# elizabethfong/SparkSmithWaterman

Hardware: NVIDIA B200
Metric: GCUPS incl. traceback (150 bp reads x 10k RefSeq-shaped refs per B200) (higher is better)
Workload: dtype s16x2

## Files before the change

sparksmithwaterman_b200/csrc/swb_trace_tile.cu:

```cuda
#include "swb_internal.h"
#include "swb_device.cuh"

#include <algorithm>
#include <cstdlib>

namespace swb {

namespace {

constexpr int NT = 128;
constexpr int TRACE_ROLL_K = 25;

template <int K> struct TileGeo {
    static constexpr int ROWW = Geo<K>::KW / 4;
    static constexpr int COLS = CB + 1;
    static constexpr int TILE_WORDS = ROWW * COLS;
    static constexpr int PROF_WORDS = 5 * GL * Geo<K>::KS;
};

template <int K>
__device__ __forceinline__ int tile_byte(const uint8_t *tile8, int rr, int cc)
{
    return tile8[(size_t)((cc * TileGeo<K>::ROWW + (rr >> 2)) * NT) * 4 + (rr & 3)];
}

template <int K>
__device__ __forceinline__ void store_col8(uint32_t *col, int top, const int (&H)[K], uint32_t k64k)
{
    constexpr int ROWW = TileGeo<K>::ROWW;
#pragma unroll
    for (int w = 0; w < ROWW; ++w) {
        const uint32_t v0 = (w == 0) ? (uint32_t)top : (uint32_t)H[4 * w - 1 < K ? 4 * w - 1 : 0];
        const uint32_t v1 = (4 * w + 0 < K) ? (uint32_t)H[4 * w + 0 < K ? 4 * w + 0 : 0] : 0u;
        const uint32_t v2 = (4 * w + 1 < K) ? (uint32_t)H[4 * w + 1 < K ? 4 * w + 1 : 0] : 0u;
        const uint32_t v3 = (4 * w + 2 < K) ? (uint32_t)H[4 * w + 2 < K ? 4 * w + 2 : 0] : 0u;
        const uint32_t p01 = v1 * k64k + ((w == 0 || 4 * w - 1 < K) ? v0 : 0u);
        const uint32_t p23 = v3 * k64k + v2;
        col[w * NT] = __byte_perm(p01, p23, 0x6420);
    }
}

__device__ __forceinline__ uint32_t prmt(uint32_t a, uint32_t b, uint32_t sel)
{
    uint32_t r;
    asm("prmt.b32 %0, %1, %2, %3;" : "=r"(r) : "r"(a), "r"(b), "r"(sel));
    return r;
}

template <int K, bool TIE_GT>
__global__ void __launch_bounds__(NT) tile_trace_kernel(const BatchParams P, const uint64_t *keys, uint32_t n_cells,
                                                        int chunk, int32_t *beginnings, int32_t *op_lens, uint32_t *ops,
                                                        int ops_stride, uint32_t k64k)
{
    using G = Geo<K>;
    using TG = TileGeo<K>;
    constexpr int KS = G::KS, ROWW = TG::ROWW;
    constexpr unsigned FULL = 0xffffffffu;
    extern __shared__ __align__(16) uint32_t smem[];
    __shared__ uint32_t seg_next;
    int *prof = reinterpret_cast<int *>(smem);
    uint32_t *tile = smem + TG::PROF_WORDS + threadIdx.x;
    const uint8_t *tile8 = reinterpret_cast<const uint8_t *>(tile);
    uint8_t *rcodes_s = reinterpret_cast<uint8_t *>(smem + TG::PROF_WORDS + (size_t)TG::TILE_WORDS * NT);
    const int gap = P.gap, match = P.match, mismatch = P.mismatch, sbias = P.seam_bias;
    const int ag = -gap;
    const uint32_t kone = k64k >> 16;

    const uint32_t c_lo = blockIdx.x * (uint32_t)chunk;
    const uint32_t c_hi = min(n_cells, c_lo + (uint32_t)chunk);
    uint32_t seg_lo = c_lo;
    while (seg_lo < c_hi) {
        const uint32_t slot = (uint32_t)(key_pair(keys[seg_lo]) / (uint64_t)P.n_refs);
        uint32_t seg_hi;
        {
            const uint64_t target = make_key((uint64_t)(slot + 1) * (uint64_t)P.n_refs, 0, 0);
            uint32_t lo = seg_lo, hi = c_hi;
            while (lo < hi) { const uint32_t mid = lo + ((hi - lo) >> 1); if (keys[mid] < target) lo = mid + 1; else hi = mid; }
            seg_hi = lo;
        }
        const int read_idx = P.rp_reads[slot];
        const int rh = (int)(slot & 1u);
        const int64_t roff = P.read_off[read_idx];
        const int m = (int)(P.read_off[read_idx + 1] - roff);
        __syncthreads();
        for (int idx = threadIdx.x; idx < 5 * GL * K; idx += NT) {
            const int cc = idx / (GL * K), rem = idx - cc * GL * K;
            const int tt = rem / K, r = rem - tt * K;
            const int row = tt * K + r;
            int s = S_PAD;
            if (row < m && cc < 4) s = ((int)P.read_codes[roff + row] == cc) ? match : mismatch;
            prof[(cc < 4 ? tt * 4 + cc : 4 * GL + tt) * KS + r] = s + ag;
        }
        for (int idx = threadIdx.x; idx < GL * K; idx += NT)
            rcodes_s[idx] = idx < m ? P.read_codes[roff + idx] : (uint8_t)0xFE;
        if (threadIdx.x == 0) seg_next = seg_lo;
        __syncthreads();

        bool busy = false;
        int ci = 0, cj = 0, n = 0;
        const uint32_t *rw = P.ref_words;
        int64_t bk = 0;
        uint32_t w_cell = 0, w_opword = 0;
        int w_h = 0, w_beg = 0, w_len = 0;

        for (;;) {
            if (!busy) {
                const uint32_t e = atomicAdd(&seg_next, 1u);
                if (e < seg_hi) {
                    const uint64_t key = keys[e];
                    const int ro = (int)(key_pair(key) - (uint64_t)slot * (uint64_t)P.n_refs);
                    const int ref = P.ref_sorted_of[ro];
                    ci = (int)key_i(key); cj = (int)key_j(key);
                    n = P.ref_len[ref];
                    rw = P.ref_words + P.ref_word_off[ref];
                    bk = (int64_t)(slot >> 1) * P.blocks_per_rp + P.ref_blk_off[ref];
                    w_cell = e; w_opword = 0; w_beg = 0; w_len = 0;
                    w_h = P.scores[(int64_t)ro * P.n_reads + read_idx];
                    busy = w_h > 0;
                    if (!busy) { beginnings[e] = 0; op_lens[e] = 0; }
                }
            }
            if (!__any_sync(FULL, busy)) break;

            const int t = busy ? (ci - 1) / K : 0;
            const int step = cj - 1 + t;
            const int b = busy ? step / CB : 0;
            int H[K], diag = 0;
            {
                load_checkpoint<K>(rec_lane<K>(P.rec, bk + b, t), busy && b > 0, [&](int w, uint32_t v) {
                    if (w < K) H[w < K ? w : 0] = half_of(v, rh); else diag = half_of(v, rh);
                });
            }
            int top[CB];
            {
                const uint32_t *sq = rec_lane<K>(P.rec, bk + b, t) + G::CKP * REC_P;
                const bool ld = busy && t > 0;
                const int bias0 = sbias * (9 - t);
#pragma unroll
                for (int p = 0; p < CB / 8; ++p) {
                    uint32_t v[8] = {0, 0, 0, 0, 0, 0, 0, 0};
                    if (ld) ldg256(sq + p * REC_P, v);
#pragma unroll
                    for (int e = 0; e < 8; ++e)
                        top[8 * p + e] = ld ? half_of(v[e], rh) - (bias0 + sbias * (8 * p + e)) : 0;
                }
            }
            uint32_t win; int ulo, uhi;
            {
                const int j0 = b * CB - t;
                const int wi = j0 >> 4;
                const uint32_t a0 = (busy && wi >= 0 && wi * 16 < n) ? __ldg(rw + wi) : 0u;
                const uint32_t a1 = (busy && wi + 1 >= 0 && (wi + 1) * 16 < n) ? __ldg(rw + wi + 1) : 0u;
                win = __funnelshift_r(a0, a1, 2 * (j0 & 15));
                ulo = -j0; uhi = busy ? n - j0 - 1 : -1;
            }
            store_col8<K>(tile, diag, H, k64k);

            const int *pbase = prof + t * 4 * KS, *ppad = prof + (4 * GL + t) * KS;
            auto column = [&](int u, int tv, uint32_t code) {
                const bool real = (u >= ulo) && (u <= uhi);
                const int *pv = real ? pbase + code * KS : ppad;
                int sv[G::KP];
                {
                    const int4 *p4 = reinterpret_cast<const int4 *>(pv);
#pragma unroll
                    for (int q = 0; q < G::KP / 4; ++q) {
                        const int4 v = p4[q];
                        sv[4 * q] = v.x; sv[4 * q + 1] = v.y; sv[4 * q + 2] = v.z; sv[4 * q + 3] = v.w;
                    }
                }
                const int floorc = ag * (u + 1);
                const int topb = tv + floorc;
                int nw = diag, nn = topb;
#pragma unroll
                for (int r = 0; r < K; ++r) {
                    const int tt = nw * (int)kone + sv[r];
                    const int pre = __vimax3_s32(tt, H[r], floorc);
                    nw = H[r];
                    H[r] = __viaddmax_s32(nn, gap, pre);
                    nn = H[r];
                }
                diag = topb;
                store_col8<K>(tile + (u + 1) * ROWW * NT, topb, H, k64k);
            };
            if constexpr (K < TRACE_ROLL_K) {
#pragma unroll
                for (int u = 0; u < CB; ++u) column(u, top[u], (win >> (2 * u)) & 3u);
            } else {
#pragma unroll 1
                for (int q = 0; q < CB / 4; ++q) {
                    int tv[4];
#pragma unroll
                    for (int e = 0; e < 4; ++e) {
                        int x = top[e];
#pragma unroll
                        for (int qq = 1; qq < CB / 4; ++qq) x = (q == qq) ? top[4 * qq + e] : x;
                        tv[e] = x;
                    }
                    const uint32_t wq = win >> (8 * q);
#pragma unroll
                    for (int e = 0; e < 4; ++e) column(4 * q + e, tv[e], (wq >> (2 * e)) & 3u);
                }
            }

            if (busy) {
                constexpr int UPB = NT * 4, COLB = ROWW * NT * 4;
                int r = ci - t * K;
                int c = step - b * CB + 1;
                const int cbase = cj - c;
                const uint8_t *pw = tile8 + (size_t)((c * ROWW + (r >> 2)) * NT) * 4;
                uint32_t sel3 = (uint32_t)(r & 3) + 3u;
                uint32_t wsh = __brev(win);
                wsh = ((wsh & 0x55555555u) << 1) | ((wsh >> 1) & 0x55555555u);
                wsh >>= 2 * (CB - c);
                const uint8_t *qp = rcodes_s + (ci - 1);
                uint32_t *op_ptr = ops + (size_t)w_cell * ops_stride + (w_len >> 4);
                uint32_t sh = 2u * ((uint32_t)w_len & 15u);
                int lastc = c;
                for (;;) {
                    const uint32_t w_c = *reinterpret_cast<const uint32_t *>(pw), u_c = *reinterpret_cast<const uint32_t *>(pw - UPB);
                    const uint32_t w_l = *reinterpret_cast<const uint32_t *>(pw - COLB), u_l = *reinterpret_cast<const uint32_t *>(pw - COLB - UPB);
                    const int hn = (int)prmt(u_c, w_c, sel3), hw = (int)prmt(u_l, w_l, sel3 + 1u), hnw = (int)prmt(u_l, w_l, sel3);
                    const int sc = ((uint32_t)*qp == (wsh & 3u)) ? match : mismatch;
                    const int whb = w_h + ag * c;
                    const bool eq_a = ((hnw + sc + ag - whb) & 0xff) == 0, eq_i = ((hn + gap - whb) & 0xff) == 0,
                               eq_d = ((hw - whb) & 0xff) == 0;
                    const uint32_t op = TIE_GT ? (eq_d ? 3u : (eq_i ? 2u : 1u)) : (eq_a ? 1u : (eq_i ? 2u : 3u));
                    lastc = c;
                    w_opword |= op << sh;
                    sh = (sh + 2u) & 31u;
                    if (sh == 0u) { *op_ptr = w_opword; w_opword = 0; }
                    op_ptr += (sh == 0u);
                    ++w_len;
                    w_h -= (op == 1u) ? sc : gap;
                    const int up = op != 3u, left = op != 2u;
                    r -= up; qp -= up; sel3 -= up;
                    if (sel3 < 3u) { sel3 = 6u; pw -= UPB; }
                    c -= left; pw -= left ? COLB : 0; wsh >>= 2 * left;
                    if (w_h <= 0 || r == 0 || c == 0) break;
                }
                ci = t * K + r; cj = cbase + c;
                w_beg = cbase + lastc;
                if (w_h <= 0) {
                    if (sh) *op_ptr = w_opword;
                    beginnings[w_cell] = w_beg;
                    op_lens[w_cell] = w_len;
                    busy = false;
                }
            }
        }
        seg_lo = seg_hi;
    }
}

template <int K> struct RowMask { using type = uint32_t; };
template <> struct RowMask<40> { using type = uint64_t; };
template <> struct RowMask<48> { using type = uint64_t; };
template <> struct RowMask<56> { using type = uint64_t; };
template <> struct RowMask<64> { using type = uint64_t; };
__device__ __forceinline__ int mask_ffs(uint32_t m) { return __ffs((int)m); }
__device__ __forceinline__ int mask_ffs(uint64_t m) { return __ffsll((long long)m); }

template <int K>
struct TileSweep {
    using mask_t = typename RowMask<K>::type;
    static_assert(K <= 8 * (int)sizeof(mask_t), "row mask too narrow for K");
    int rc[K], H[K];
    int diag, S, t, b;
    uint32_t win;
    mask_t rowok;
    int ulo, uhi;
    const uint32_t *sq;
    bool has_top;
    uint64_t pkey;
    int64_t pair;

    __device__ __forceinline__ void setup(const BatchParams &P, const TileTask &T, bool live)
    {
        using G = Geo<K>;
        const int rp = (int)(T.rp_half >> 1), rh = (int)(T.rp_half & 1u), ref = (int)T.ref_sorted;
        t = (int)T.lane; b = (int)T.block;
        S = 0x7fffffff; pkey = 0; pair = 0; diag = 0; win = 0; rowok = 0; ulo = 0; uhi = -1;
        sq = P.rec; has_top = false;
#pragma unroll
        for (int r = 0; r < K; ++r) { rc[r] = 0xFE; H[r] = 0; }
        if (!live) return;
        const int read_idx = P.rp_reads[2 * rp + rh];
        const int64_t off = P.read_off[read_idx];
        const int m = (int)(P.read_off[read_idx + 1] - off);
        const int n = P.ref_len[ref];
        const int64_t ro = P.ref_orig[ref];
        pair = ro * P.n_reads + read_idx;
        S = P.scores[pair];
        pkey = (uint64_t)T.rp_half * (uint64_t)P.n_refs + (uint64_t)ro;
#pragma unroll
        for (int r = 0; r < K; ++r) {
            const int row = t * K + r;
            rc[r] = (row < m) ? (int)P.read_codes[off + row] : 0xFE;
            if (row < m) rowok |= (mask_t)1 << r;
        }
        const int64_t blk = (int64_t)rp * P.blocks_per_rp + P.ref_blk_off[ref] + b;
        if (b > 0) {
            load_checkpoint<K>(rec_lane<K>(P.rec, blk, t), true, [&](int w, uint32_t v) {
                if (w < K) H[w < K ? w : 0] = half_of(v, rh); else diag = half_of(v, rh);
            });
        }
        sq = rec_lane<K>(P.rec, blk, t) + G::CKP * REC_P;
        has_top = t > 0;
        const uint32_t *rw = P.ref_words + P.ref_word_off[ref];
        const int j0 = b * CB - t;
        const int wi = j0 >> 4;
        const uint32_t a0 = (wi >= 0 && wi * 16 < n) ? __ldg(rw + wi) : 0u;
        const uint32_t a1 = (wi + 1 >= 0 && (wi + 1) * 16 < n) ? __ldg(rw + wi + 1) : 0u;
        win = __funnelshift_r(a0, a1, 2 * (j0 & 15));
        ulo = -j0; uhi = n - j0 - 1;
        (void)rh;
    }

    template <class Fn>
    __device__ __forceinline__ void run(const BatchParams &P, int rh, Fn &&fn)
    {
        const int gap = P.gap, match = P.match, mismatch = P.mismatch;
        const int bias0 = P.seam_bias * (9 - t);
        uint32_t sv[CB];
#pragma unroll
        for (int p = 0; p < CB / 8; ++p) {
            uint32_t v[8] = {0, 0, 0, 0, 0, 0, 0, 0};
            if (has_top) ldg256(sq + p * REC_P, v);
#pragma unroll
            for (int e = 0; e < 8; ++e) sv[8 * p + e] = v[e];
        }
#pragma unroll 1
        for (int q = 0; q < CB / 4; ++q) {
            uint32_t av[4];
#pragma unroll
            for (int e = 0; e < 4; ++e) {
                uint32_t x = sv[e];
#pragma unroll
                for (int qq = 1; qq < CB / 4; ++qq) x = (q == qq) ? sv[4 * qq + e] : x;
                av[e] = x;
            }
#pragma unroll
            for (int e = 0; e < 4; ++e) {
                const int u = 4 * q + e;
                const int top = has_top ? half_of(av[e], rh) - (bias0 + P.seam_bias * u) : 0;
                const bool real = (u >= ulo) && (u <= uhi);
                const int c = real ? (int)((win >> (2 * u)) & 3u) : 0xFD;
                int nw = diag, nn = top, cmax = 0;
#pragma unroll
                for (int r = 0; r < K; ++r) {
                    const int sc = (rc[r] == c) ? match : mismatch;
                    const int x = __viaddmax_s32_relu(nw, sc, 0);
                    const int pre = __viaddmax_s32(H[r], gap, x);
                    nw = H[r];
                    H[r] = real ? __viaddmax_s32(nn, gap, pre) : 0;
                    nn = H[r];
                    cmax = max(cmax, H[r]);
                }
                diag = top;
                if (real) fn(b * CB - t + u + 1, cmax, H);
            }
        }
    }
};

struct TileHit { int32_t emax; uint32_t n; uint32_t code[4]; };

template <int K>
__global__ void __launch_bounds__(NT) tile_scan_kernel(const BatchParams P, const TileTask *tasks,
                                                       const uint32_t *n_tasks_ptr, uint32_t cap_tasks, TileHit *hits)
{
    __shared__ uint32_t hitbuf[4 * NT];
    const uint32_t n_tasks = min(*n_tasks_ptr, cap_tasks);
    const uint32_t n_threads = gridDim.x * blockDim.x;
    for (uint32_t task = blockIdx.x * blockDim.x + threadIdx.x; task < n_tasks; task += n_threads) {
        const TileTask T = tasks[task];
        TileSweep<K> W;
        W.setup(P, T, true);
        int E = max(W.S, 1);
        uint32_t n_hit = 0;
        const int t = W.t;
        using mask_t = typename TileSweep<K>::mask_t;
        const mask_t rowok = W.rowok;
        W.run(P, (int)(T.rp_half & 1u), [&](int j, int cmax, const int (&H)[K]) {
            if (cmax < E) return;
            int vm = 0;
#pragma unroll
            for (int r = 0; r < K; ++r) vm = max(vm, ((rowok >> r) & 1u) ? H[r] : 0);
            if (vm < E) return;
            if (vm > E) { E = vm; n_hit = 0; }
            mask_t rm = 0;
#pragma unroll
            for (int r = 0; r < K; ++r) rm |= (H[r] == E) ? ((mask_t)1 << r) : (mask_t)0;
            rm &= rowok;
            while (rm) {
                const int r = mask_ffs(rm) - 1;
                rm &= rm - 1;
                if (n_hit < 4) hitbuf[n_hit * NT + threadIdx.x] = ((uint32_t)(t * K + r + 1) << KEY_J_BITS) | (uint32_t)j;
                ++n_hit;
            }
        });
        if (n_hit && E > W.S) atomicMax(P.scores + W.pair, E);
        TileHit o;
        o.emax = n_hit ? E : 0; o.n = n_hit;
#pragma unroll
        for (int h = 0; h < 4; ++h) o.code[h] = (uint32_t)h < n_hit ? hitbuf[h * NT + threadIdx.x] : 0u;
        hits[task] = o;
    }
}

template <int K, bool SEL>
__global__ void __launch_bounds__(NT) tile_emit_kernel(const BatchParams P, const TileTask *tasks,
                                                       const uint32_t *n_tasks_ptr, uint32_t cap_tasks, const TileHit *hits,
                                                       uint64_t *keys, uint32_t cap, uint32_t *count)
{
    const uint32_t n_tasks = min(*n_tasks_ptr, cap_tasks);
    const int lane = threadIdx.x & 31;
    const uint32_t n_threads = gridDim.x * blockDim.x;
    const uint32_t iters = (n_tasks + n_threads - 1) / n_threads;
    for (uint32_t it = 0; it < iters; ++it) {
        const uint32_t task = it * n_threads + blockIdx.x * blockDim.x + threadIdx.x;
        const bool live = task < n_tasks;
        TileTask T = TileTask{0, 0, 0, 0};
        TileHit h; h.emax = 0; h.n = 0;
        uint64_t pkey = 0;
        bool hot = false;
        if (live) {
            T = tasks[task];
            h = hits[task];
            const int read_idx = P.rp_reads[T.rp_half];
            const int64_t ro = P.ref_orig[T.ref_sorted];
            pkey = ((uint64_t)T.rp_half * (uint64_t)P.n_refs + (uint64_t)ro) << (KEY_J_BITS + KEY_I_BITS);
            hot = h.n > 0 && h.emax == P.scores[ro * P.n_reads + read_idx];
            if (SEL) {
                const uint64_t b = (uint64_t)T.rp_half * (uint64_t)P.n_refs + (uint64_t)ro;
                hot = hot && ((P.sel[b >> 5] >> (b & 31)) & 1u);
            }
        }
        const uint32_t mine = hot ? min(h.n, 4u) : 0u;
        uint32_t inc = mine;
#pragma unroll
        for (int o = 1; o < 32; o <<= 1) { const uint32_t v = __shfl_up_sync(0xffffffffu, inc, o); if (lane >= o) inc += v; }
        const uint32_t total = __shfl_sync(0xffffffffu, inc, 31);
        uint32_t base = 0;
        if (lane == 31 && total) base = atomicAdd(count, total);
        base = __shfl_sync(0xffffffffu, base, 31) + inc - mine;
        if (hot && h.n <= 4) {
#pragma unroll
            for (int k = 0; k < 4; ++k)
                if ((uint32_t)k < mine && base + k < cap) keys[base + k] = pkey | h.code[k];
        } else if (hot) {
            TileSweep<K> W;
            W.setup(P, T, true);
            const int S = h.emax;
            const int t = W.t;
            using mask_t = typename TileSweep<K>::mask_t;
            const mask_t rowok = W.rowok;
            uint32_t seen = 0;
            W.run(P, (int)(T.rp_half & 1u), [&](int j, int cmax, const int (&H)[K]) {
                if (cmax < S) return;
                mask_t rm = 0;
#pragma unroll
                for (int r = 0; r < K; ++r) rm |= (H[r] == S) ? ((mask_t)1 << r) : (mask_t)0;
                rm &= rowok;
                while (rm) {
                    const int r = mask_ffs(rm) - 1;
                    rm &= rm - 1;
                    const uint32_t k = seen < 4 ? base + seen : atomicAdd(count, 1u);
                    ++seen;
                    if (k < cap) keys[k] = pkey | ((uint32_t)(t * K + r + 1) << KEY_J_BITS) | (uint32_t)j;
                }
            });
        }
    }
}

template <int K>
cudaError_t launch_tile_locate_k(const BatchParams &P, const TileTask *tasks, const uint32_t *n_tasks, uint32_t cap_tasks,
                                 void *hits, uint64_t *keys, uint32_t cap, uint32_t *count, int sm_count, int phase, cudaStream_t st)
{
    const int64_t ctas = std::max<int64_t>(1, std::min<int64_t>(((int64_t)cap_tasks + NT - 1) / NT, (int64_t)sm_count * 32));
    if (phase == 0) tile_scan_kernel<K><<<(unsigned)ctas, NT, 0, st>>>(P, tasks, n_tasks, cap_tasks, static_cast<TileHit *>(hits));
    else if (P.sel) tile_emit_kernel<K, true><<<(unsigned)ctas, NT, 0, st>>>(P, tasks, n_tasks, cap_tasks, static_cast<const TileHit *>(hits), keys, cap, count);
    else tile_emit_kernel<K, false><<<(unsigned)ctas, NT, 0, st>>>(P, tasks, n_tasks, cap_tasks, static_cast<const TileHit *>(hits), keys, cap, count);
    return cudaGetLastError();
}

template <int K>
cudaError_t launch_tile_trace_k(const BatchParams &P, const uint64_t *keys, uint32_t n_cells, int32_t *beginnings,
                                int32_t *op_lens, uint32_t *ops, int ops_stride, int sm_count, cudaStream_t st)
{
    using TG = TileGeo<K>;
    if (n_cells == 0) return cudaSuccess;
    const size_t smem = ((size_t)TG::PROF_WORDS + (size_t)TG::TILE_WORDS * NT) * sizeof(uint32_t) + (((size_t)GL * K + 15) / 16) * 16;
    static PerDeviceOnce attr;
    {
        const cudaError_t e = attr.run([&] {
            cudaError_t e1 = cudaFuncSetAttribute(tile_trace_kernel<K, false>, cudaFuncAttributeMaxDynamicSharedMemorySize, (int)smem);
            if (e1 == cudaSuccess) e1 = cudaFuncSetAttribute(tile_trace_kernel<K, true>, cudaFuncAttributeMaxDynamicSharedMemorySize, (int)smem);
            return e1;
        });
        if (e != cudaSuccess) return e;
    }
    const int per_sm = 16;
    const int chunk = (int)std::max<int64_t>(P.sel ? 1 : 2 * NT, ((int64_t)n_cells + (int64_t)sm_count * per_sm - 1) / ((int64_t)sm_count * per_sm));
    const int64_t ctas = ((int64_t)n_cells + chunk - 1) / chunk;
    if (P.tie_gt) tile_trace_kernel<K, true><<<(unsigned)ctas, NT, smem, st>>>(P, keys, n_cells, chunk, beginnings, op_lens, ops, ops_stride, 65536u);
    else          tile_trace_kernel<K, false><<<(unsigned)ctas, NT, smem, st>>>(P, keys, n_cells, chunk, beginnings, op_lens, ops, ops_stride, 65536u);
    return cudaGetLastError();
}

}

bool tile_trace_ok(int match, int mismatch, int gap)
{
    if (gap >= 0) return false;
    const int64_t smax = std::max<int64_t>({match, mismatch, 0});
    const int64_t sabs = std::max<int64_t>(std::llabs((long long)match), std::llabs((long long)mismatch));
    return 2 * (smax - (int64_t)gap) + sabs < 250;
}

size_t locate_hit_bytes() { return sizeof(TileHit); }

cudaError_t launch_locate(int K, const BatchParams &P, const TileTask *tasks, const uint32_t *n_tasks,
                          uint32_t cap_tasks, void *hits, uint64_t *keys, uint32_t cap, uint32_t *count, int sm_count,
                          int phase, cudaStream_t st)
{
    switch (K) {
        case 4:  return launch_tile_locate_k<4>(P, tasks, n_tasks, cap_tasks, hits, keys, cap, count, sm_count, phase, st);
        case 5:  return launch_tile_locate_k<5>(P, tasks, n_tasks, cap_tasks, hits, keys, cap, count, sm_count, phase, st);
        case 7:  return launch_tile_locate_k<7>(P, tasks, n_tasks, cap_tasks, hits, keys, cap, count, sm_count, phase, st);
        case 10: return launch_tile_locate_k<10>(P, tasks, n_tasks, cap_tasks, hits, keys, cap, count, sm_count, phase, st);
        case 8:  return launch_tile_locate_k<8>(P, tasks, n_tasks, cap_tasks, hits, keys, cap, count, sm_count, phase, st);
        case 13: return launch_tile_locate_k<13>(P, tasks, n_tasks, cap_tasks, hits, keys, cap, count, sm_count, phase, st);
        case 16: return launch_tile_locate_k<16>(P, tasks, n_tasks, cap_tasks, hits, keys, cap, count, sm_count, phase, st);
        case 19: return launch_tile_locate_k<19>(P, tasks, n_tasks, cap_tasks, hits, keys, cap, count, sm_count, phase, st);
        case 25: return launch_tile_locate_k<25>(P, tasks, n_tasks, cap_tasks, hits, keys, cap, count, sm_count, phase, st);
        case 32: return launch_tile_locate_k<32>(P, tasks, n_tasks, cap_tasks, hits, keys, cap, count, sm_count, phase, st);
        case 40: return launch_tile_locate_k<40>(P, tasks, n_tasks, cap_tasks, hits, keys, cap, count, sm_count, phase, st);
        case 48: return launch_tile_locate_k<48>(P, tasks, n_tasks, cap_tasks, hits, keys, cap, count, sm_count, phase, st);
        case 56: return launch_tile_locate_k<56>(P, tasks, n_tasks, cap_tasks, hits, keys, cap, count, sm_count, phase, st);
        case 64: return launch_tile_locate_k<64>(P, tasks, n_tasks, cap_tasks, hits, keys, cap, count, sm_count, phase, st);
    }
    return cudaErrorInvalidValue;
}

cudaError_t launch_tile_trace(int K, const BatchParams &P, const uint64_t *keys, uint32_t n_cells, int32_t *beginnings,
                              int32_t *op_lens, uint32_t *ops, int ops_stride_words, int sm_count, cudaStream_t st)
{
    switch (K) {
        case 4:  return launch_tile_trace_k<4>(P, keys, n_cells, beginnings, op_lens, ops, ops_stride_words, sm_count, st);
        case 5:  return launch_tile_trace_k<5>(P, keys, n_cells, beginnings, op_lens, ops, ops_stride_words, sm_count, st);
        case 7:  return launch_tile_trace_k<7>(P, keys, n_cells, beginnings, op_lens, ops, ops_stride_words, sm_count, st);
        case 10: return launch_tile_trace_k<10>(P, keys, n_cells, beginnings, op_lens, ops, ops_stride_words, sm_count, st);
        case 8:  return launch_tile_trace_k<8>(P, keys, n_cells, beginnings, op_lens, ops, ops_stride_words, sm_count, st);
        case 13: return launch_tile_trace_k<13>(P, keys, n_cells, beginnings, op_lens, ops, ops_stride_words, sm_count, st);
        case 16: return launch_tile_trace_k<16>(P, keys, n_cells, beginnings, op_lens, ops, ops_stride_words, sm_count, st);
        case 19: return launch_tile_trace_k<19>(P, keys, n_cells, beginnings, op_lens, ops, ops_stride_words, sm_count, st);
        case 25: return launch_tile_trace_k<25>(P, keys, n_cells, beginnings, op_lens, ops, ops_stride_words, sm_count, st);
        case 32: return launch_tile_trace_k<32>(P, keys, n_cells, beginnings, op_lens, ops, ops_stride_words, sm_count, st);
        case 40: return launch_tile_trace_k<40>(P, keys, n_cells, beginnings, op_lens, ops, ops_stride_words, sm_count, st);
        case 48: return launch_tile_trace_k<48>(P, keys, n_cells, beginnings, op_lens, ops, ops_stride_words, sm_count, st);
        case 56: return launch_tile_trace_k<56>(P, keys, n_cells, beginnings, op_lens, ops, ops_stride_words, sm_count, st);
        case 64: return launch_tile_trace_k<64>(P, keys, n_cells, beginnings, op_lens, ops, ops_stride_words, sm_count, st);
    }
    return cudaErrorInvalidValue;
}

}
```

Baseline: 9920.

## Pack two row halves into s16x2 SIMD lanes in tile traceback fill

For K up to MAX_K_BASE, the traceback tile fill now splits each thread's K rows into two halves and computes them together in packed 16-bit lanes, using vmax3/viaddmax. The upper half lags the lower by TRACE_LAG columns, fed through ring buffers, so the dependency chain is roughly halved. The score profile is rebuilt as a pair-indexed packed table with a rotated bank layout, and byte-permute plans reassemble tile bytes from the packed registers. It also adds minimum-CTA launch bounds per K. The cost is extra skew iterations, a larger profile table in shared memory, more complex packing code, and possible register pressure.

```diff
diff --git a/sparksmithwaterman_b200/csrc/swb_trace_tile.cu b/sparksmithwaterman_b200/csrc/swb_trace_tile.cu
--- a/sparksmithwaterman_b200/csrc/swb_trace_tile.cu
+++ b/sparksmithwaterman_b200/csrc/swb_trace_tile.cu
@@ -10,13 +10,95 @@
 
 constexpr int NT = 128;
 constexpr int TRACE_ROLL_K = 25;
+constexpr int TRACE_LAG = 4;
 
 template <int K> struct TileGeo {
     static constexpr int ROWW = Geo<K>::KW / 4;
     static constexpr int COLS = CB + 1;
     static constexpr int TILE_WORDS = ROWW * COLS;
-    static constexpr int PROF_WORDS = 5 * GL * Geo<K>::KS;
+    static constexpr bool PACKED = K <= MAX_K_BASE;
+    static constexpr int KH = (K + 1) / 2;
+    static constexpr int NQ = (KH + 3) / 4;
+    static constexpr int PROF_WORDS = PACKED ? 25 * NQ * GL * 4 : 5 * GL * Geo<K>::KS;
 };
+
+struct PackPlan {
+    int kind[2], ra[2], ba[2], rb[2], bb[2];
+    int ppos[4];
+    bool merged;
+    int pos[4];
+};
+
+template <int K>
+__host__ __device__ constexpr PackPlan pack_plan(int w, bool want_low, bool want_high)
+{
+    constexpr int KH = TileGeo<K>::KH;
+    int reg[4] = {0, 0, 0, 0}, byt[4] = {0, 0, 0, 0};
+    bool care[4] = {false, false, false, false};
+    for (int k = 0; k < 4; ++k) {
+        const int rho = 4 * w + k;
+        const bool low = rho <= KH;
+        care[k] = rho <= K && (low ? want_low : want_high);
+        reg[k] = rho == 0 ? -1 : (low ? rho - 1 : rho - 1 - KH);
+        byt[k] = low ? 0 : 2;
+    }
+    for (int p = 0; p < 2; ++p) {
+        const int a = 2 * p, b = 2 * p + 1;
+        if (!care[a] && care[b]) { reg[a] = reg[b]; byt[a] = byt[b]; care[a] = true; }
+        if (care[a] && !care[b]) { reg[b] = reg[a]; byt[b] = byt[a]; care[b] = true; }
+    }
+    for (int p = 0; p < 2; ++p) {
+        const int o = 2 - 2 * p;
+        if (!care[2 * p]) { reg[2 * p] = reg[o]; byt[2 * p] = byt[o]; reg[2 * p + 1] = reg[o + 1]; byt[2 * p + 1] = byt[o + 1]; }
+    }
+    PackPlan pl{};
+    for (int p = 0; p < 2; ++p) {
+        const int a = 2 * p, b = 2 * p + 1;
+        pl.ra[p] = reg[a]; pl.ba[p] = byt[a]; pl.rb[p] = reg[b]; pl.bb[p] = byt[b];
+        if (reg[a] == reg[b]) { pl.kind[p] = 0; pl.ppos[a] = byt[a]; pl.ppos[b] = byt[b]; }
+        else if (reg[a] >= 0 && reg[b] == reg[a] + 1 && byt[a] == byt[b]) { pl.kind[p] = 1; pl.ppos[a] = byt[a]; pl.ppos[b] = byt[a] + 1; }
+        else { pl.kind[p] = 2; pl.ppos[a] = 0; pl.ppos[b] = 1; }
+    }
+    const bool same = pl.kind[0] == pl.kind[1] && pl.ra[0] == pl.ra[1] &&
+                      (pl.kind[0] != 2 || (pl.rb[0] == pl.rb[1] && pl.ba[0] == pl.ba[1] && pl.bb[0] == pl.bb[1]));
+    pl.merged = !same;
+    for (int k = 0; k < 4; ++k) pl.pos[k] = pl.merged ? k : pl.ppos[k];
+    return pl;
+}
+
+__host__ __device__ constexpr uint32_t sel4(int p0, int p1, int p2, int p3)
+{
+    return (uint32_t)p0 | ((uint32_t)p1 << 4) | ((uint32_t)p2 << 8) | ((uint32_t)p3 << 12);
+}
+
+template <int KH>
+__device__ __forceinline__ uint32_t pk_reg(const uint32_t (&Hp)[KH], uint32_t nn0, int i)
+{
+    return i < 0 ? nn0 : Hp[i < 0 ? 0 : i];
+}
+
+template <int KH>
+__device__ __forceinline__ uint32_t pk_piece(const PackPlan &pl, int p, const uint32_t (&Hp)[KH], uint32_t nn0)
+{
+    const uint32_t a = pk_reg(Hp, nn0, pl.ra[p]);
+    if (pl.kind[p] == 0) return a;
+    if (pl.kind[p] == 1) return __byte_perm(a, pk_reg(Hp, nn0, pl.ra[p] + 1), 0x6240);
+    return __byte_perm(a, pk_reg(Hp, nn0, pl.rb[p]), sel4(pl.ba[p], 4 + pl.bb[p], 0, 0));
+}
+
+template <int KH>
+__device__ __forceinline__ uint32_t gather(const PackPlan &pl, const uint32_t (&Hp)[KH], uint32_t nn0)
+{
+    const uint32_t v0 = pk_piece(pl, 0, Hp, nn0);
+    if (!pl.merged) return v0;
+    return __byte_perm(v0, pk_piece(pl, 1, Hp, nn0), sel4(pl.ppos[0], pl.ppos[1], 4 + pl.ppos[2], 4 + pl.ppos[3]));
+}
+
+__device__ __forceinline__ uint32_t place(const PackPlan &pl, uint32_t v)
+{
+    const bool ident = pl.pos[0] == 0 && pl.pos[1] == 1 && pl.pos[2] == 2 && pl.pos[3] == 3;
+    return ident ? v : __byte_perm(v, v, sel4(pl.pos[0], pl.pos[1], pl.pos[2], pl.pos[3]));
+}
 
 template <int K>
 __device__ __forceinline__ int tile_byte(const uint8_t *tile8, int rr, int cc)
@@ -47,8 +129,10 @@
     return r;
 }
 
+constexpr int trace_min_ctas(int K) { return K <= 5 ? 9 : K <= 10 ? 8 : K <= 13 ? 7 : K <= 19 ? 6 : K <= MAX_K_BASE ? 4 : 0; }
+
 template <int K, bool TIE_GT>
-__global__ void __launch_bounds__(NT) tile_trace_kernel(const BatchParams P, const uint64_t *keys, uint32_t n_cells,
+__global__ void __launch_bounds__(NT, trace_min_ctas(K)) tile_trace_kernel(const BatchParams P, const uint64_t *keys, uint32_t n_cells,
                                                         int chunk, int32_t *beginnings, int32_t *op_lens, uint32_t *ops,
                                                         int ops_stride, uint32_t k64k)
 {
@@ -83,13 +167,26 @@
         const int64_t roff = P.read_off[read_idx];
         const int m = (int)(P.read_off[read_idx + 1] - roff);
         __syncthreads();
-        for (int idx = threadIdx.x; idx < 5 * GL * K; idx += NT) {
-            const int cc = idx / (GL * K), rem = idx - cc * GL * K;
-            const int tt = rem / K, r = rem - tt * K;
-            const int row = tt * K + r;
-            int s = S_PAD;
-            if (row < m && cc < 4) s = ((int)P.read_codes[roff + row] == cc) ? match : mismatch;
-            prof[(cc < 4 ? tt * 4 + cc : 4 * GL + tt) * KS + r] = s + ag;
+        if constexpr (TG::PACKED) {
+            for (int idx = threadIdx.x; idx < TG::PROF_WORDS; idx += NT) {
+                const int e = idx & 3, rest = idx >> 5;
+                const int pair = rest / TG::NQ, i = 4 * (rest - pair * TG::NQ) + e;
+                const int tt = ((idx >> 2) - pair) & (GL - 1);
+                const int cl = pair / 5, ch = pair - 5 * cl;
+                const int rl = tt * K + i, rhw = rl + TG::KH;
+                const int sl = (i < TG::KH && cl < 4 && rl < m) ? (((int)P.read_codes[roff + rl] == cl) ? match : mismatch) + ag : 0;
+                const int sh = (i + TG::KH < K && ch < 4 && rhw < m) ? (((int)P.read_codes[roff + rhw] == ch) ? match : mismatch) + ag : 0;
+                smem[idx] = ((uint32_t)sh << 16) + (uint32_t)sl;
+            }
+        } else {
+            for (int idx = threadIdx.x; idx < 5 * GL * K; idx += NT) {
+                const int cc = idx / (GL * K), rem = idx - cc * GL * K;
+                const int tt = rem / K, r = rem - tt * K;
+                const int row = tt * K + r;
+                int s = S_PAD;
+                if (row < m && cc < 4) s = ((int)P.read_codes[roff + row] == cc) ? match : mismatch;
+                prof[(cc < 4 ? tt * 4 + cc : 4 * GL + tt) * KS + r] = s + ag;
+            }
         }
         for (int idx = threadIdx.x; idx < GL * K; idx += NT)
             rcodes_s[idx] = idx < m ? P.read_codes[roff + idx] : (uint8_t)0xFE;
@@ -156,6 +253,95 @@
             }
             store_col8<K>(tile, diag, H, k64k);
 
+            if constexpr (TG::PACKED) {
+                constexpr int KH = TG::KH, NQ = TG::NQ;
+                constexpr int OFF = 256;
+                const uint4 *tab = reinterpret_cast<const uint4 *>(smem);
+                const uint32_t g2 = pack2(gap, gap);
+                constexpr int LAG = TRACE_LAG, NIT = CB + LAG;
+                const uint32_t fl0 = pack2(ag + OFF, ag * (1 - LAG) + OFF), fl1 = pack2(ag, ag);
+                uint32_t Hp[KH], Hck[KH], hist[LAG], carry[LAG];
+#pragma unroll
+                for (int i = 0; i < KH; ++i) {
+                    Hp[i] = pack2(H[i] + OFF, (i + KH < K ? H[i + KH < K ? i + KH : 0] : 0) + OFF);
+                    Hck[i] = Hp[i];
+                }
+#pragma unroll
+                for (int k = 0; k < LAG; ++k) { hist[k] = Hp[KH - 1]; carry[k] = 0; }
+                uint32_t dg = (uint32_t)(diag + OFF);
+                auto iter = [&](int u, int ph, int tv) {
+                    const int uh = u - LAG;
+                    const bool rlo = u < CB && u >= ulo && u <= uhi, rhi = uh >= 0 && uh >= ulo && uh <= uhi;
+                    const int cl = rlo ? (int)((win >> (2 * u)) & 3u) : 4;
+                    const int ch = rhi ? (int)((win >> (2 * uh)) & 3u) : 4;
+                    const int pair = cl * 5 + ch;
+                    const uint4 *pv = tab + pair * (NQ * GL) + ((t + pair) & (GL - 1));
+                    uint32_t sv[4 * NQ];
+#pragma unroll
+                    for (int q = 0; q < NQ; ++q) {
+                        const uint4 v = pv[q * GL];
+                        sv[4 * q] = v.x; sv[4 * q + 1] = v.y; sv[4 * q + 2] = v.z; sv[4 * q + 3] = v.w;
+                    }
+                    const uint32_t floorv = fl1 * (uint32_t)u + fl0;
+                    const int ph1 = (ph + 1) & (LAG - 1);
+                    const uint32_t nn0 = __byte_perm((uint32_t)(tv + ag * (u + 1) + OFF), hist[ph1], 0x5410);
+                    uint32_t nw = dg, nn = nn0;
+#pragma unroll
+                    for (int r = 0; r < KH; ++r) {
+                        const uint32_t tt = nw * kone + sv[r];
+                        const uint32_t pre = vmax3(tt, Hp[r], floorv);
+                        nw = Hp[r];
+                        Hp[r] = viaddmax(nn, g2, pre);
+                        nn = Hp[r];
+                    }
+                    dg = nn0;
+                    hist[ph1] = Hp[KH - 1];
+                    if (u == LAG - 1) {
+#pragma unroll
+                        for (int i = 0; i < KH; ++i) Hp[i] = __byte_perm(Hp[i], Hck[i], 0x7610);
+                    }
+                    uint32_t *colL = tile + (u + 1) * ROWW * NT, *colH = tile + (uh + 1) * ROWW * NT;
+#pragma unroll
+                    for (int w = 0; w < ROWW; ++w) {
+                        const bool has_lo = 4 * w <= KH, has_hi = 4 * w + 3 > KH;
+                        if (has_lo && !has_hi) {
+                            if (u < CB) { const PackPlan pl = pack_plan<K>(w, true, false); colL[w * NT] = place(pl, gather(pl, Hp, nn0)); }
+                        } else if (has_hi && !has_lo) {
+                            if (uh >= 0) { const PackPlan pl = pack_plan<K>(w, false, true); colH[w * NT] = place(pl, gather(pl, Hp, nn0)); }
+                        } else {
+                            const PackPlan pl = pack_plan<K>(w, true, false), ph2 = pack_plan<K>(w, false, true);
+                            if (uh >= 0) {
+                                const uint32_t hv = gather(ph2, Hp, nn0);
+                                uint32_t s[4];
+#pragma unroll
+                                for (int k = 0; k < 4; ++k) s[k] = 4 * w + k <= KH ? pl.pos[k] : 4 + ph2.pos[k];
+                                colH[w * NT] = __byte_perm(carry[ph], hv, sel4(s[0], s[1], s[2], s[3]));
+                            }
+                            if (u < CB) carry[ph] = gather(pl, Hp, nn0);
+                        }
+                    }
+                };
+                if constexpr (K < TRACE_ROLL_K) {
+#pragma unroll
+                    for (int u = 0; u < NIT; ++u) iter(u, u & (LAG - 1), u < CB ? top[u < CB ? u : 0] : 0);
+                } else {
+                    static_assert(4 % LAG == 0, "a quad of iterations must hold whole turns of the LAG-slot rings");
+#pragma unroll 1
+                    for (int q = 0; q < (NIT + 3) / 4; ++q) {
+                        int tv[4];
+#pragma unroll
+                        for (int e = 0; e < 4; ++e) {
+                            int x = top[e];
+#pragma unroll
+                            for (int qq = 1; qq < CB / 4; ++qq) x = (q == qq) ? top[4 * qq + e] : x;
+                            tv[e] = q < CB / 4 ? x : 0;
+                        }
+#pragma unroll
+                        for (int e = 0; e < 4; ++e)
+                            if (NIT % 4 == 0 || 4 * q + e < NIT) iter(4 * q + e, e & (LAG - 1), tv[e]);
+                    }
+                }
+            } else {
             const int *pbase = prof + t * 4 * KS, *ppad = prof + (4 * GL + t) * KS;
             auto column = [&](int u, int tv, uint32_t code) {
                 const bool real = (u >= ulo) && (u <= uhi);
@@ -201,6 +387,7 @@
 #pragma unroll
                     for (int e = 0; e < 4; ++e) column(4 * q + e, tv[e], (wq >> (2 * e)) & 3u);
                 }
+            }
             }
 
             if (busy) {
```

Measured after the change: 9604 (median of 6 runs). 0.968x the previous value.
